# luisdavid64/MRI-Implicit-Neural-Representations

Measured on AMD Instinct MI355X. Metric: coord-samples/sec (fwd+bwd) fitting 640x368x15-coil k-space; PSNR@1k steps, higher is better.
Workload: dtype f32; 1 GPU; SIREN 5x256 gauss-512 k-space fit, synthetic 640x368x15-coil, L2, Adam; batch_per_gpu=25000, global_batch=25000, parallelism=single, launch=eager

## Files before the change

mri-implicit-neural-representations_amd/csrc/inr_mlp_rs_impl.h:

```cpp
#pragma once
#include "inr_mlp_impl.h"

namespace inr {

constexpr int RS_PITCH = 132;
constexpr int RS_IMG_FLOATS = 256 * RS_PITCH;
constexpr int RS_CP = 32;
constexpr int RS_CHUNK_FLOATS = 2 * RS_CP * RS_PITCH;
constexpr int RS_CHUNK_STEPS = 2 * RS_CP / 4;
constexpr int RS_PF = 8;
constexpr int RS_LR = 8;
constexpr int RS_OOB = 0x7ffffff0;
constexpr int RS_HSZ = 256 * 128;

typedef float f32x2 __attribute__((ext_vector_type(2)));
typedef unsigned u32x2 __attribute__((ext_vector_type(2)));
typedef __attribute__((address_space(3))) float lfloat;
typedef __attribute__((address_space(3))) f32x4 lf32x4;

__device__ __forceinline__ f32x4 mfma16(float a, float b, f32x4 c) {
  return __builtin_amdgcn_mfma_f32_16x16x4f32(a, b, c, 0, 0, 0);
}

template <int NCB>
__device__ __forceinline__ int rs_tl(int c, int jj) {
  return ((NCB & 1) && c == NCB - 1) ? 16 * (NCB - 1) + jj : 32 * (c >> 1) + 2 * jj + (c & 1);
}
template <int NCB>
__device__ __forceinline__ bool rs_active(int c, int n) {
  return ((NCB & 1) && c == NCB - 1) ? n == NCB : (c | 1) < n;
}

template <int NCB>
struct RsAddr {
  static constexpr int NP = (NCB + 1) / 2;
  __amdgpu_buffer_rsrc_t rs;
  int cB[NP];
  int cC[NP];
};

__device__ __forceinline__ void rs_store2(__amdgpu_buffer_rsrc_t rs, int voff, int soff, float x, float y) {
  u32x2 v = {__builtin_bit_cast(unsigned, x), __builtin_bit_cast(unsigned, y)};
  __builtin_amdgcn_raw_buffer_store_b64(v, rs, voff, soff, 0);
}
__device__ __forceinline__ void rs_store1(__amdgpu_buffer_rsrc_t rs, int voff, int soff, float x) {
  __builtin_amdgcn_raw_buffer_store_b32(__builtin_bit_cast(unsigned, x), rs, voff, soff, 0);
}
__device__ __forceinline__ f32x2 rs_load2(__amdgpu_buffer_rsrc_t rs, int voff, int soff) {
  return __builtin_bit_cast(f32x2, __builtin_amdgcn_raw_buffer_load_b64(rs, voff, soff, 0));
}
__device__ __forceinline__ float rs_load1(__amdgpu_buffer_rsrc_t rs, int voff, int soff) {
  return __builtin_bit_cast(float, __builtin_amdgcn_raw_buffer_load_b32(rs, voff, soff, 0));
}

__device__ __forceinline__ float rs_dk_put(bool in_agpr, float v) {
  if (!in_agpr) return v;
  float a;
  asm("v_accvgpr_write_b32 %0, %1" : "=a"(a) : "v"(v));
  return a;
}
__device__ __forceinline__ float rs_dk_get(bool in_agpr, float a) {
  if (!in_agpr) return a;
  float v;
  asm("v_accvgpr_read_b32 %0, %1" : "=v"(v) : "a"(a));
  return v;
}
template <int NCB>
constexpr bool rs_dk_agpr(int rb, int reg) { return true; }

__device__ __forceinline__ float rs_bval(const f32x4& b0, const f32x4& b1, int c) { return c < 4 ? b0[c] : b1[c - 4]; }

template <int NCB>
__device__ __forceinline__ void rs_store_brows(const RsAddr<NCB>& ad, int soff, const f32x4& b0, const f32x4& b1) {
  constexpr int NP = RsAddr<NCB>::NP;
#pragma unroll
  for (int p = 0; p < NP; ++p) {
    if ((NCB & 1) && p == NP - 1)
      rs_store1(ad.rs, ad.cB[p], soff, rs_bval(b0, b1, 2 * p));
    else
      rs_store2(ad.rs, ad.cB[p], soff, rs_bval(b0, b1, 2 * p), rs_bval(b0, b1, 2 * p + 1));
  }
}

template <int NCB>
__device__ __forceinline__ void rs_store_crow(const RsAddr<NCB>& ad, int soff, const f32x4 (&v)[2]) {
  constexpr int NP = RsAddr<NCB>::NP;
#pragma unroll
  for (int p = 0; p < NP; ++p) {
    if ((NCB & 1) && p == NP - 1)
      rs_store1(ad.rs, ad.cC[p], soff, v[(2 * p) >> 2][(2 * p) & 3]);
    else
      rs_store2(ad.rs, ad.cC[p], soff, v[(2 * p) >> 2][(2 * p) & 3], v[(2 * p + 1) >> 2][(2 * p + 1) & 3]);
  }
}

#define RS_KIND_FEAT 1
#define RS_KIND_FWD 2
#define RS_KIND_BWD 3

template <int NCB, int NSTEPS, int KIND, int INIT>
__device__ __forceinline__ void rs_gemm(f32x4 (&acc)[4][NCB], f32x4 (&Ar)[RS_PF], const __amdgpu_buffer_rsrc_t ars,
                                        const int avoff, const int asoff, const int asoff_next, const lfloat* Bl,
                                        const RsAddr<NCB>& ad, const int w, const int soffB, const int soffB2,
                                        f32x2 (&dk)[4][4][(NCB + 1) / 2], const int soffD, const f32x4 (&cinit)[4]) {
  constexpr int NP = (NCB + 1) / 2;
  constexpr int NQ = (NCB + 3) / 4;
  static_assert(NSTEPS % RS_PF == 0, "the fragment ring must be in phase at the start of every GEMM");
  f32x2 lr[RS_LR];
  f32x4 b0, b1 = {0.f, 0.f, 0.f, 0.f};
  b0 = *(const lf32x4*)(Bl);
  if (NQ > 1) b1 = *(const lf32x4*)(Bl + 4);
  const lfloat* Blw = Bl + w * 4 * RS_PITCH;
  f32x4 st0, st1 = {0.f, 0.f, 0.f, 0.f};
  st0 = *(const lf32x4*)(Blw);
  if (NQ > 1) st1 = *(const lf32x4*)(Blw + 4);
#pragma unroll
  for (int s = 0; s < NSTEPS; ++s) {
    const f32x4 afr = Ar[s % RS_PF];
    {
      const int so = s + RS_PF < NSTEPS ? asoff + (s + RS_PF) * 4096 : asoff_next + (s + RS_PF - NSTEPS) * 4096;
      Ar[s % RS_PF] = __builtin_bit_cast(f32x4, __builtin_amdgcn_raw_buffer_load_b128(ars, avoff, so, 0));
    }
    f32x4 n0 = b0, n1 = b1;
    if (s + 1 < NSTEPS) {
      n0 = *(const lf32x4*)(Bl + (s + 1) * 4 * RS_PITCH);
      if (NQ > 1) n1 = *(const lf32x4*)(Bl + (s + 1) * 4 * RS_PITCH + 4);
    }
    if ((s & 3) == 0) {
      const int rowb = KIND == RS_KIND_FEAT ? (s < NSTEPS / 2 ? soffB + 4 * s * 512 : soffB2 + 4 * (s - NSTEPS / 2) * 512)
                                            : soffB + 4 * s * 512;
      rs_store_brows<NCB>(ad, rowb + w * 2048, st0, st1);
    }
    if ((s & 3) == 3 && s + 1 < NSTEPS) {
      st0 = *(const lf32x4*)(Blw + (s + 1) * 4 * RS_PITCH);
      if (NQ > 1) st1 = *(const lf32x4*)(Blw + (s + 1) * 4 * RS_PITCH + 4);
    }
    if (KIND == RS_KIND_FWD || KIND == RS_KIND_BWD) {
      constexpr int TOT = 16 * NP;
      const int j0 = s * TOT / NSTEPS, j1 = (s + 1) * TOT / NSTEPS;
#pragma unroll
      for (int j = j0; j < j1; ++j) {
        const int rr = j / NP, p = j % NP, rb = rr >> 2, reg = rr & 3;
        const int so = soffD + (16 * rb + reg) * 512;
        const bool single = (NCB & 1) && p == NP - 1;
        if (KIND == RS_KIND_FWD) {
          if (single)
            rs_store1(ad.rs, ad.cC[p], so, rs_dk_get(rs_dk_agpr<NCB>(rb, reg), dk[rb][reg][p][0]));
          else
            rs_store2(ad.rs, ad.cC[p], so, rs_dk_get(rs_dk_agpr<NCB>(rb, reg), dk[rb][reg][p][0]),
                      rs_dk_get(rs_dk_agpr<NCB>(rb, reg), dk[rb][reg][p][1]));
        } else {
          if (j >= RS_LR) {
            const int jo = j - RS_LR, ro = jo / NP, po = jo % NP;
            dk[ro >> 2][ro & 3][po][0] = rs_dk_put(rs_dk_agpr<NCB>(ro >> 2, ro & 3), lr[jo % RS_LR][0]);
            if (!((NCB & 1) && po == NP - 1))
              dk[ro >> 2][ro & 3][po][1] = rs_dk_put(rs_dk_agpr<NCB>(ro >> 2, ro & 3), lr[jo % RS_LR][1]);
          }
          if (single) {
            lr[j % RS_LR][0] = rs_load1(ad.rs, ad.cC[p], so);
            lr[j % RS_LR][1] = 0.f;
          } else {
            lr[j % RS_LR] = rs_load2(ad.rs, ad.cC[p], so);
          }
        }
      }
    }
#pragma unroll
    for (int c = 0; c < NCB; ++c) {
      const float bv = rs_bval(b0, b1, c);
#pragma unroll
      for (int rb = 0; rb < 4; ++rb)
        acc[rb][c] = mfma16(afr[rb], bv,
                            (INIT == 1 && s == 0) ? f32x4{0.f, 0.f, 0.f, 0.f} : ((INIT == 2 && s == 0) ? cinit[rb] : acc[rb][c]));
    }
#pragma unroll
    for (int i = 0; i < 12; ++i) {
      __builtin_amdgcn_sched_group_barrier(0x008, 1, 0);
      __builtin_amdgcn_sched_group_barrier(0x1b6, 1, 0);
    }
    __builtin_amdgcn_sched_barrier(0);
    b0 = n0;
    b1 = n1;
  }
  if (KIND == RS_KIND_BWD) {
    constexpr int TOT = 16 * NP;
#pragma unroll
    for (int jo = TOT - RS_LR; jo < TOT; ++jo) {
      const int ro = jo / NP, po = jo % NP;
      dk[ro >> 2][ro & 3][po][0] = rs_dk_put(rs_dk_agpr<NCB>(ro >> 2, ro & 3), lr[jo % RS_LR][0]);
      if (!((NCB & 1) && po == NP - 1))
        dk[ro >> 2][ro & 3][po][1] = rs_dk_put(rs_dk_agpr<NCB>(ro >> 2, ro & 3), lr[jo % RS_LR][1]);
    }
  }
}

template <int NCB>
__device__ __forceinline__ void rs_gen(lfloat* buf, const lfloat* encB_lds, int ch, const float (&xs)[NCB][3], int tid) {
  const int jj = tid & 15, p0 = tid >> 4;
#pragma unroll
  for (int i = 0; i < 2; ++i) {
    const int p = p0 + 16 * i, s = ch * RS_CP + p;
    const float e0 = encB_lds[3 * s + 0], e1 = encB_lds[3 * s + 1], e2 = encB_lds[3 * s + 2];
    f32x4 sn[2] = {{0.f, 0.f, 0.f, 0.f}, {0.f, 0.f, 0.f, 0.f}}, cs[2] = {{0.f, 0.f, 0.f, 0.f}, {0.f, 0.f, 0.f, 0.f}};
#pragma unroll
    for (int c = 0; c < NCB; ++c) {
      const float ph = fmaf(xs[c][2], e2, fmaf(xs[c][1], e1, xs[c][0] * e0));
      float a, b;
      sincos_cw(ph, a, b);
      sn[c >> 2][c & 3] = a;
      cs[c >> 2][c & 3] = b;
    }
    lfloat* q = buf + p * RS_PITCH + jj * 8;
    *(lf32x4*)(q) = sn[0];
    *(lf32x4*)(q + RS_CP * RS_PITCH) = cs[0];
    if (NCB > 4) {
      *(lf32x4*)(q + 4) = sn[1];
      *(lf32x4*)(q + RS_CP * RS_PITCH + 4) = cs[1];
    }
  }
}

template <int HACT>
__device__ __forceinline__ float rs_act_park(float z, float w0, float& h) {
  if (HACT == ACT_SIN) {
    constexpr float c_hi = 0.15915494309189535f;
    constexpr float c_lo = (float)(0.15915494309189533576888 - (double)c_hi);
    const float t = w0 * z;
    const float k = rintf(t * c_hi);
    const float rev = fmaf(t, c_lo, fmaf(t, c_hi, -k));
    h = __builtin_amdgcn_sinf(rev);
    return rev;
  }
  float d;
  act_fwd<HACT>(z, w0, h, d);
  return z;
}
template <int HACT>
__device__ __forceinline__ void rs_act_unpark(float p, float w0, float& h, float& d) {
  if (HACT == ACT_SIN) {
    h = __builtin_amdgcn_sinf(p);
    d = w0 * __builtin_amdgcn_cosf(p);
  } else {
    act_fwd<HACT>(p, w0, h, d);
  }
}

template <int NCB, int HACT>
struct RsLast {
  lfloat *wl_lds, *dzl, *red, *part, *Cl;
  float* slab;
  bool lvalid, sampled, first;
  long long lrow;
  int w, kq, jj, tid, lane;

  template <int MO>
  __device__ __forceinline__ float run(const NetDesc& nd, const LossDesc& ld, const MlpArgs& a, const f32x4 (&acc)[4][NCB],
                                       const float (&gt_pre)[4], const float (&lb_pre)[4], float w0) {
    constexpr int NQ = (NCB + 3) / 4;
    constexpr int NW = 4;
    (void)NW;
    const LayerDesc& LL = nd.L[nd.D - 1];
    float loss = 0.f;
    f32x4 yp[MO][2];
#pragma unroll
    for (int o = 0; o < MO; ++o) yp[o][0] = yp[o][1] = f32x4{0.f, 0.f, 0.f, 0.f};
#pragma unroll
    for (int rb = 0; rb < 4; ++rb) {
      f32x4 wv[MO];
#pragma unroll
      for (int o = 0; o < MO; ++o) wv[o] = *(const lf32x4*)(wl_lds + o * 256 + 64 * w + 16 * rb + 4 * kq);
#pragma unroll
      for (int reg = 0; reg < 4; ++reg) {
        f32x4 hq[2] = {{0.f, 0.f, 0.f, 0.f}, {0.f, 0.f, 0.f, 0.f}}, pq[2] = {{0.f, 0.f, 0.f, 0.f}, {0.f, 0.f, 0.f, 0.f}};
#pragma unroll
        for (int c = 0; c < NCB; ++c) {
          float h;
          pq[c >> 2][c & 3] = rs_act_park<HACT>(acc[rb][c][reg], w0, h);
          hq[c >> 2][c & 3] = h;
        }
#pragma unroll
        for (int q = 0; q < NQ; ++q) {
          *(lf32x4*)(Cl + (16 * rb + reg) * RS_PITCH + 4 * q) = pq[q];
#pragma unroll
          for (int o = 0; o < MO; ++o) yp[o][q] += wv[o][reg] * hq[q];
        }
        __builtin_amdgcn_sched_barrier(0);
      }
    }
    INR_STAMP(50);
#pragma unroll
    for (int o = 0; o < MO; ++o)
#pragma unroll
      for (int q = 0; q < 2; ++q)
#pragma unroll
        for (int e = 0; e < 4; ++e) {
          float v = yp[o][q][e];
          v += __shfl_xor(v, 16);
          v += __shfl_xor(v, 32);
          yp[o][q][e] = v;
        }
    if (kq == 0) {
#pragma unroll
      for (int o = 0; o < MO; ++o) {
        lfloat* pp = part + (w * MO + o) * 128 + jj * 8;
        *(lf32x4*)pp = yp[o][0];
        *(lf32x4*)(pp + 4) = yp[o][1];
      }
    }
    INR_STAMP(51);
    __syncthreads();
    INR_STAMP(52);
    if (tid < 128) {
      float zl[4], y[4], dy[4], g[4] = {0.f, 0.f, 0.f, 0.f}, dz[4] = {0.f, 0.f, 0.f, 0.f};
#pragma unroll
      for (int o = 0; o < 4; ++o) {
        float s = 0.f;
        if (o < MO)
          s = ((part[o * 128 + tid] + part[(MO + o) * 128 + tid]) + part[(2 * MO + o) * 128 + tid]) +
              part[(3 * MO + o) * 128 + tid];
        zl[o] = o < nd.out_f ? s + lb_pre[o] : 0.f;
      }
      const int nrows = nd.out_f;
#pragma unroll
      for (int o = 0; o < 4; ++o) {
        y[o] = dy[o] = 0.f;
        if (o < nd.out_f) act_fwd_rt(nd.last_act, zl[o], nd.w0, y[o], dy[o]);
      }
      if (lvalid) {
#pragma unroll
        for (int o = 0; o < 4; ++o)
          if (o < nd.out_f && a.out != nullptr) a.out[lrow * nd.out_f + o] = y[o];
        if (sampled) loss = loss_row(ld, nd.out_f, y, gt_pre, g);
#pragma unroll
        for (int o = 0; o < 4; ++o)
          if (o < nrows) dz[o] = g[o] * dy[o];
      }
#pragma unroll
      for (int o = 0; o < MO; ++o) dzl[o * 128 + tid] = dz[o];
    }
    INR_STAMP(53);
    __syncthreads();
    INR_STAMP(54);
    f32x4 dzv[MO][2];
#pragma unroll
    for (int o = 0; o < MO; ++o)
#pragma unroll
      for (int q = 0; q < 2; ++q)
        dzv[o][q] = q < NQ ? *(const lf32x4*)(dzl + o * 128 + jj * 8 + 4 * q) : f32x4{0.f, 0.f, 0.f, 0.f};
    const __amdgpu_buffer_rsrc_t rsb = uniform_rsrc(slab + LL.gb_off, LL.M * 4);
    float db_mine, dw_mine[4];
    {
      float sb[MO];
#pragma unroll
      for (int o = 0; o < MO; ++o) {
        sb[o] = 0.f;
#pragma unroll
        for (int c = 0; c < NCB; ++c) sb[o] += dzv[o][c >> 2][c & 3];
      }
      group_sum_n<16, MO>(sb);
      float mine = sb[0];
#pragma unroll
      for (int o = 1; o < MO; ++o) mine = jj == o ? sb[o] : mine;
      db_mine = mine;
    }
    const __amdgpu_buffer_rsrc_t rsw = uniform_rsrc(slab + LL.gw_off, LL.M * LL.K * 4);
    {
      f32x4 nx[2] = {{0.f, 0.f, 0.f, 0.f}, {0.f, 0.f, 0.f, 0.f}};
#pragma unroll
      for (int q = 0; q < NQ; ++q) nx[q] = *(const lf32x4*)(Cl + 4 * q);
      f32x4 wv[MO];
      float pw[MO * 4];
#pragma unroll
      for (int rr = 0; rr < 16; ++rr) {
        const int rb = rr >> 2, reg = rr & 3;
        lfloat* row = Cl + (16 * rb + reg) * RS_PITCH;
        if (reg == 0) {
#pragma unroll
          for (int o = 0; o < MO; ++o) wv[o] = *(const lf32x4*)(wl_lds + o * 256 + 64 * w + 16 * rb + 4 * kq);
        }
        f32x4 hq[2] = {nx[0], nx[1]}, dq[2] = {{0.f, 0.f, 0.f, 0.f}, {0.f, 0.f, 0.f, 0.f}};
        f32x4 dd[2] = {{0.f, 0.f, 0.f, 0.f}, {0.f, 0.f, 0.f, 0.f}};
        if (rr + 1 < 16) {
#pragma unroll
          for (int q = 0; q < NQ; ++q)
            nx[q] = *(const lf32x4*)(Cl + (16 * ((rr + 1) >> 2) + ((rr + 1) & 3)) * RS_PITCH + 4 * q);
        }
#pragma unroll
        for (int c = 0; c < NCB; ++c) {
          float h, d;
          rs_act_unpark<HACT>(hq[c >> 2][c & 3], w0, h, d);
          hq[c >> 2][c & 3] = h;
          dd[c >> 2][c & 3] = d;
        }
#pragma unroll
        for (int o = 0; o < MO; ++o) {
          float sp = 0.f;
#pragma unroll
          for (int c = 0; c < NCB; ++c) sp = fmaf(dzv[o][c >> 2][c & 3], hq[c >> 2][c & 3], sp);
          pw[o * 4 + reg] = sp;
        }
#pragma unroll
        for (int c = 0; c < NCB; ++c) {
          float sd = 0.f;
#pragma unroll
          for (int o = 0; o < MO; ++o) sd = fmaf(wv[o][reg], dzv[o][c >> 2][c & 3], sd);
          dq[c >> 2][c & 3] = sd * dd[c >> 2][c & 3];
        }
#pragma unroll
        for (int q = 0; q < NQ; ++q) *(lf32x4*)(row + 4 * q) = dq[q];
        if (reg == 3) {
          group_sum_n<16, MO * 4>(pw);
          float mine = pw[0];
#pragma unroll
          for (int i = 1; i < MO * 4; ++i) mine = jj == i ? pw[i] : mine;
          dw_mine[rb] = mine;
        }
        __builtin_amdgcn_sched_barrier(0);
      }
    }
    {
      const int so_ = jj >> 2;
      int off[5];
#pragma unroll
      for (int rb = 0; rb < 4; ++rb) {
        const int rowi = 64 * w + 16 * rb + 4 * kq + (jj & 3);
        off[rb] = (jj < MO * 4 && so_ < LL.M && rowi < LL.K) ? (so_ * LL.K + rowi) * 4 : RS_OOB;
      }
      off[4] = (w == 0 && kq == 0 && jj < MO && jj < LL.M) ? jj * 4 : RS_OOB;
      if (!first) {
        float old[5];
#pragma unroll
        for (int rb = 0; rb < 4; ++rb) old[rb] = rs_load1(rsw, off[rb], 0);
        old[4] = rs_load1(rsb, off[4], 0);
#pragma unroll
        for (int rb = 0; rb < 4; ++rb) dw_mine[rb] += old[rb];
        db_mine += old[4];
      }
#pragma unroll
      for (int rb = 0; rb < 4; ++rb) rs_store1(rsw, off[rb], 0, dw_mine[rb]);
      rs_store1(rsb, off[4], 0, db_mine);
    }
    INR_STAMP(55);
    return loss;
  }
};

template <int NCB, int HACT>
__global__ __launch_bounds__(256) void inr_mlp_rs_kernel(const NetDesc nd, const LossDesc ld, const MlpArgs a) {
  extern __shared__ __attribute__((aligned(16))) float lds[];
  constexpr int NW = 4;
  (void)NW;
  constexpr int NP = (NCB + 1) / 2;
  constexpr int NQ = (NCB + 3) / 4;
  const int tid = threadIdx.x, lane = tid & 63;
  const int w = __builtin_amdgcn_readfirstlane(tid >> 6);
  INR_RT_STAMP(a.dbg, a.dbg_cap, NW, w, lane, 44);
  const int kq = lane >> 4, jj = lane & 15;
  const int D = nd.D, E = nd.E;
  lfloat* img = (lfloat*)lds;
  lfloat* encB_lds = img + RS_IMG_FLOATS;
  lfloat* wl_lds = encB_lds + ((3 * E + 3) & ~3);
  lfloat* dzl = wl_lds + 1024;
  lfloat* red = dzl + 512;
  lfloat* part = red + 32;
  const LayerDesc& LL = nd.L[D - 1];
  for (int i = tid; i < 3 * E; i += 256) encB_lds[i] = a.encB[i];
  for (int i = tid; i < 1024; i += 256) {
    const int o = i >> 8, k = i & 255;
    wl_lds[i] = (o < LL.M && k < LL.K) ? a.params[LL.w_off + o * LL.K + k] : 0.f;
  }
  float* slab = a.slabs + (size_t)blockIdx.x * nd.slab_floats;
  float loss_acc = 0.f;
  if (((int)blockIdx.x < a.rs_x ? a.rs_hi : a.rs_lo) == 0 && a.accumulate == 0) {
    for (int i = tid; i < LL.M * LL.K; i += 256) slab[LL.gw_off + i] = 0.f;
    if (tid < LL.M) slab[LL.gb_off + tid] = 0.f;
  }
  const long long spt = nd.save_floats_per_tile;
  const __amdgpu_buffer_rsrc_t ars = uniform_rsrc(a.packed, 0x7ffffff0);
  const int avoff = lane * 16 + w * 1024;
  const lfloat* Bl = img + kq * RS_PITCH + jj * 8;
  lfloat* Cl = img + (64 * w + 4 * kq) * RS_PITCH + jj * 8;
  const int enc_off = (2 * (D - 1) * RS_HSZ + 4 * 128) * 4;
  const int nch = E / RS_CP;
  f32x4 Ar[RS_PF];
  {
    const int so = nd.L[0].rf_off * 4;
#pragma unroll
    for (int i = 0; i < RS_PF; ++i)
      Ar[i] = __builtin_bit_cast(f32x4, __builtin_amdgcn_raw_buffer_load_b128(ars, avoff, so + i * 4096, 0));
  }

  for (int r = 0; r < a.rs_rounds; ++r) {
    const int t = r * gridDim.x + blockIdx.x;
    const int n = t < a.rs_x ? a.rs_hi : a.rs_lo;
    const int blk0 = t < a.rs_x ? t * a.rs_hi : a.rs_x * a.rs_hi + (t - a.rs_x) * a.rs_lo;
    if (n == 0) continue;
    const bool first = r == 0 && a.accumulate == 0;
    const long long g0 = (long long)blk0 * 16;
    const int slot0 = blk0 >> 3;
    RsAddr<NCB> ad;
    {
      const int nslots = a.n_tiles - slot0 < 2 ? a.n_tiles - slot0 : 2;
      ad.rs = uniform_rsrc(a.save + (size_t)slot0 * spt, (int)(nslots * spt * 4));
#pragma unroll
      for (int p = 0; p < NP; ++p) {
        const int gl = (blk0 & 7) * 16 + rs_tl<NCB>(2 * p, jj);
        const int off = (int)(((gl >> 7) * spt + (gl & 127)) * 4);
        const bool act = rs_active<NCB>(2 * p, n);
        ad.cB[p] = act ? off + kq * 512 : RS_OOB;
        ad.cC[p] = act ? off + kq * 2048 : RS_OOB;
      }
    }
    float xs[NCB][3];
#pragma unroll
    for (int c = 0; c < NCB; ++c) {
      const long long g = g0 + rs_tl<NCB>(c, jj);
      const bool ok = rs_active<NCB>(c, n) && g < a.B;
      const float two_pi = 6.283185307179586f;
#pragma unroll
      for (int i = 0; i < 3; ++i) xs[c][i] = ok ? two_pi * a.x[3 * g + i] : 0.f;
    }
    float gt_pre[4] = {0.f, 0.f, 0.f, 0.f}, lb_pre[4] = {0.f, 0.f, 0.f, 0.f};
    bool sampled_pre = false, lvalid = false;
    long long lrow = 0;
    if (tid < 128) {
      const int cq = tid & 7, jq = tid >> 3;
      if (cq < NCB) {
        lrow = g0 + rs_tl<NCB>(cq, jq);
        lvalid = rs_active<NCB>(cq, n) && lrow < a.B;
      }
#pragma unroll
      for (int o = 0; o < 4; ++o)
        if (o < nd.out_f) lb_pre[o] = a.packed[LL.pbias_off + o];
      if (lvalid) {
        sampled_pre = a.mask == nullptr || a.mask[lrow] != 0;
#pragma unroll
        for (int o = 0; o < 4; ++o)
          if (o < nd.out_f) gt_pre[o] = a.gt[lrow * nd.out_f + o];
      }
    }
    INR_STAMP(0);
    __syncthreads();
    f32x4 acc[4][NCB];
    f32x2 dk[4][4][NP];
    f32x4 bnext[4];
#pragma unroll
    for (int rb = 0; rb < 4; ++rb) {
      bnext[rb] = *reinterpret_cast<const f32x4*>(a.packed + nd.L[0].pbias_off + 64 * w + 4 * kq + 16 * rb);
#pragma unroll
      for (int c = 0; c < NCB; ++c) acc[rb][c] = bnext[rb];
    }
    rs_gen<NCB>(img, encB_lds, 0, xs, tid);
    __syncthreads();
    for (int ch = 0; ch < nch; ++ch) {
      if (ch == 1) INR_STAMP(56);
      if (ch + 1 < nch) rs_gen<NCB>(img + ((ch + 1) & 1) * RS_CHUNK_FLOATS, encB_lds, ch + 1, xs, tid);
      if (ch == 1) INR_STAMP(57);
      const int ao = (nd.L[0].rf_off + ch * RS_CHUNK_STEPS * 1024) * 4;
      const int an = ch + 1 < nch ? ao + RS_CHUNK_STEPS * 4096 : (D > 2 ? nd.L[1].rf_off : nd.L[0].rf_off) * 4;
      const int sb = enc_off + ch * RS_CP * 512;
      rs_gemm<NCB, RS_CHUNK_STEPS, RS_KIND_FEAT, 0>(acc, Ar, ars, avoff, ao, an, Bl + (ch & 1) * RS_CHUNK_FLOATS, ad, w, sb,
                                                    sb + E * 512, dk, 0, bnext);
      if (ch == 1) INR_STAMP(58);
      __syncthreads();
      if (ch == 1) INR_STAMP(59);
    }
    INR_STAMP(1);
    for (int l = 1; l <= D - 2; ++l) {
      {
#pragma unroll
        for (int rb = 0; rb < 4; ++rb)
          bnext[rb] = *reinterpret_cast<const f32x4*>(a.packed + nd.L[l].pbias_off + 64 * w + 4 * kq + 16 * rb);
        const float w0 = nd.L[l - 1].omega;
#pragma unroll
        for (int rb = 0; rb < 4; ++rb) {
#pragma unroll
          for (int reg = 0; reg < 4; ++reg) {
            f32x4 hq[2] = {{0.f, 0.f, 0.f, 0.f}, {0.f, 0.f, 0.f, 0.f}};
#pragma unroll
            for (int c = 0; c < NCB; ++c) {
              float h, d;
              act_fwd<HACT>(acc[rb][c][reg], w0, h, d);
              hq[c >> 2][c & 3] = h;
              dk[rb][reg][c >> 1][c & 1] = rs_dk_put(rs_dk_agpr<NCB>(rb, reg), d);
            }
#pragma unroll
            for (int q = 0; q < NQ; ++q) *(lf32x4*)(Cl + (16 * rb + reg) * RS_PITCH + 4 * q) = hq[q];
            __builtin_amdgcn_sched_barrier(0);
          }
        }
      }
      if (l == 1) INR_STAMP(60);
      __syncthreads();
      INR_STAMP(20 + l - 1);
      const LayerDesc& Ll = nd.L[l];
      const int an = l < D - 2 ? nd.L[l + 1].rf_off * 4 : nd.L[D - 2].rb_off * 4;
      rs_gemm<NCB, 64, RS_KIND_FWD, 2>(acc, Ar, ars, avoff, Ll.rf_off * 4, an, Bl, ad, w, (2 * (l - 1)) * RS_HSZ * 4, 0, dk,
                                       ((2 * (l - 1) + 1) * RS_HSZ + 64 * w * 128) * 4, bnext);
      INR_STAMP(1 + l);
      __syncthreads();
      if (l == 1) INR_STAMP(61);
    }
    INR_STAMP(10);
    {
      RsLast<NCB, HACT> ls{wl_lds, dzl, red, part, Cl, slab, lvalid, sampled_pre, first, lrow, w, kq, jj, tid, lane};
      if (LL.M > 2)
        loss_acc += ls.template run<4>(nd, ld, a, acc, gt_pre, lb_pre, nd.L[D - 2].omega);
      else
        loss_acc += ls.template run<2>(nd, ld, a, acc, gt_pre, lb_pre, nd.L[D - 2].omega);
    }
    __syncthreads();
    INR_STAMP(20 + D - 2);
    INR_STAMP(11);
    for (int l = D - 2; l >= 1; --l) {
      const LayerDesc& Ll = nd.L[l];
      const int an = (l > 1 ? nd.L[l - 1].rb_off : nd.L[0].rf_off) * 4;
      rs_gemm<NCB, 64, RS_KIND_BWD, 1>(acc, Ar, ars, avoff, Ll.rb_off * 4, an, Bl, ad, w, (2 * l + 1) * RS_HSZ * 4, 0, dk,
                                       ((2 * (l - 1) + 1) * RS_HSZ + 64 * w * 128) * 4, bnext);
      INR_STAMP(12 + l);
      if (l > 1) {
        __syncthreads();
#pragma unroll
        for (int rb = 0; rb < 4; ++rb)
#pragma unroll
          for (int reg = 0; reg < 4; ++reg) {
            f32x4 dq[2] = {{0.f, 0.f, 0.f, 0.f}, {0.f, 0.f, 0.f, 0.f}};
#pragma unroll
            for (int c = 0; c < NCB; ++c) dq[c >> 2][c & 3] = acc[rb][c][reg] * rs_dk_get(rs_dk_agpr<NCB>(rb, reg), dk[rb][reg][c >> 1][c & 1]);
#pragma unroll
            for (int q = 0; q < NQ; ++q) *(lf32x4*)(Cl + (16 * rb + reg) * RS_PITCH + 4 * q) = dq[q];
          }
        __syncthreads();
        INR_STAMP(30 + l);
      }
    }
    {
      const int so0 = (1 * RS_HSZ + 64 * w * 128) * 4;
#pragma unroll
      for (int rb = 0; rb < 4; ++rb)
#pragma unroll
        for (int reg = 0; reg < 4; ++reg) {
          f32x4 dq[2] = {{0.f, 0.f, 0.f, 0.f}, {0.f, 0.f, 0.f, 0.f}};
          if (D > 2) {
#pragma unroll
            for (int c = 0; c < NCB; ++c) dq[c >> 2][c & 3] = acc[rb][c][reg] * rs_dk_get(rs_dk_agpr<NCB>(rb, reg), dk[rb][reg][c >> 1][c & 1]);
          } else {
#pragma unroll
            for (int q = 0; q < NQ; ++q) dq[q] = *(const lf32x4*)(Cl + (16 * rb + reg) * RS_PITCH + 4 * q);
          }
          rs_store_crow<NCB>(ad, so0 + (16 * rb + reg) * 512, dq);
        }
    }
    INR_STAMP(40);
  }

  {
    float v = loss_acc;
#pragma unroll
    for (int off = 32; off >= 1; off >>= 1) v += __shfl_xor(v, off);
    __syncthreads();
    if (lane == 0) red[w] = v;
    __syncthreads();
    if (tid == 0) {
      const float tsum = ((red[0] + red[1]) + red[2]) + red[3];
      slab[nd.slab_loss_off] = a.accumulate ? slab[nd.slab_loss_off] + tsum : tsum;
    }
  }
  INR_RT_STAMP(a.dbg, a.dbg_cap, NW, w, lane, 45);
}

inline size_t rs_lds_bytes(const NetDesc& nd) {
  return ((size_t)RS_IMG_FLOATS + ((3 * (size_t)nd.E + 3) & ~(size_t)3) + 1024 + 512 + 32 + 2048) * sizeof(float);
}

template <int NCB, int HACT>
inline hipError_t launch_mlp_rs(const NetDesc& nd, const LossDesc& ld, const MlpArgs& a, int grid, hipStream_t st) {
  const size_t lds_bytes = rs_lds_bytes(nd);
  if (lds_bytes > 160 * 1024) return hipErrorInvalidValue;
  hipError_t e = allow_full_lds<inr_mlp_rs_kernel<NCB, HACT>>();
  if (e != hipSuccess) return e;
  hipLaunchKernelGGL((inr_mlp_rs_kernel<NCB, HACT>), dim3(grid), dim3(256), lds_bytes, st, nd, ld, a);
  return hipGetLastError();
}

}
```

Measured before the change: 61.45 million coord-samples/s.

## Interleave Fourier feature generation into layer-0 MFMA loop

Moves the sin/cos Gaussian-feature generation for the next chunk out of a separate rs_gen pass and into the layer-0 GEMM step loop. Each step computes a share of the features and writes them into the other LDS buffer, with scheduling barriers that pair MFMAs with VALU/LDS ops so transcendental work hides under matrix ops. On the last chunk it harmlessly regenerates the current chunk into the spare buffer. It adds register pressure and more complex scheduling inside the hot GEMM, which may reduce occupancy or disturb the tuned pipeline.

```diff
diff --git a/mri-implicit-neural-representations_amd/csrc/inr_mlp_rs_impl.h b/mri-implicit-neural-representations_amd/csrc/inr_mlp_rs_impl.h
--- a/mri-implicit-neural-representations_amd/csrc/inr_mlp_rs_impl.h
+++ b/mri-implicit-neural-representations_amd/csrc/inr_mlp_rs_impl.h
@@ -98,14 +98,39 @@
 #define RS_KIND_FWD 2
 #define RS_KIND_BWD 3
 
-template <int NCB, int NSTEPS, int KIND, int INIT>
+template <int NCB>
+struct RsGen {
+  int other;
+  const lfloat* enc;
+  float xs[NCB][3];
+};
+
+__device__ __forceinline__ void rs_feat(const float (&x)[3], float e0, float e1, float e2, float& sn, float& cs) {
+  const float ph = fmaf(x[2], e2, fmaf(x[1], e1, x[0] * e0));
+  sincos_cw(ph, sn, cs);
+}
+
+template <int NCB, int NSTEPS, int KIND, int INIT, bool GEN = false>
 __device__ __forceinline__ void rs_gemm(f32x4 (&acc)[4][NCB], f32x4 (&Ar)[RS_PF], const __amdgpu_buffer_rsrc_t ars,
                                         const int avoff, const int asoff, const int asoff_next, const lfloat* Bl,
                                         const RsAddr<NCB>& ad, const int w, const int soffB, const int soffB2,
-                                        f32x2 (&dk)[4][4][(NCB + 1) / 2], const int soffD, const f32x4 (&cinit)[4]) {
+                                        f32x2 (&dk)[4][4][(NCB + 1) / 2], const int soffD, const f32x4 (&cinit)[4],
+                                        const RsGen<NCB>* gen = nullptr) {
   constexpr int NP = (NCB + 1) / 2;
   constexpr int NQ = (NCB + 3) / 4;
   static_assert(NSTEPS % RS_PF == 0, "the fragment ring must be in phase at the start of every GEMM");
+  static_assert(!GEN || KIND == RS_KIND_FEAT, "only layer 0 generates features");
+  float ge[2][3] = {{0.f, 0.f, 0.f}, {0.f, 0.f, 0.f}};
+  f32x4 gsn = {0.f, 0.f, 0.f, 0.f}, gcs = {0.f, 0.f, 0.f, 0.f};
+  if (GEN) {
+    int gl;
+    asm volatile("v_mbcnt_lo_u32_b32 %0, -1, 0\n\tv_mbcnt_hi_u32_b32 %0, -1, %0" : "=v"(gl));
+    const lfloat* ep = gen->enc + 3 * (4 * w + (gl >> 4));
+#pragma unroll
+    for (int i = 0; i < 2; ++i)
+#pragma unroll
+      for (int k = 0; k < 3; ++k) ge[i][k] = ep[3 * 16 * i + k];
+  }
   f32x2 lr[RS_LR];
   f32x4 b0, b1 = {0.f, 0.f, 0.f, 0.f};
   b0 = *(const lf32x4*)(Bl);
@@ -165,6 +190,24 @@
         }
       }
     }
+    if (GEN) {
+      constexpr int TOT = 2 * NCB, GS = NSTEPS - 1;
+      const int u0 = s < GS ? s * TOT / GS : TOT, u1 = s + 1 < GS ? (s + 1) * TOT / GS : TOT;
+#pragma unroll
+      for (int u = u0; u < u1; ++u) {
+        const int i = u / NCB, c = u % NCB;
+        if ((c & 3) == 0) gsn = gcs = f32x4{0.f, 0.f, 0.f, 0.f};
+        float sn, cs;
+        rs_feat(gen->xs[c], ge[i][0], ge[i][1], ge[i][2], sn, cs);
+        gsn[c & 3] = sn;
+        gcs[c & 3] = cs;
+        if ((c & 3) == 3 || c == NCB - 1) {
+          lfloat* q = (lfloat*)Blw + gen->other + 16 * i * RS_PITCH + (c & ~3);
+          *(lf32x4*)(q) = gsn;
+          *(lf32x4*)(q + RS_CP * RS_PITCH) = gcs;
+        }
+      }
+    }
 #pragma unroll
     for (int c = 0; c < NCB; ++c) {
       const float bv = rs_bval(b0, b1, c);
@@ -173,10 +216,18 @@
         acc[rb][c] = mfma16(afr[rb], bv,
                             (INIT == 1 && s == 0) ? f32x4{0.f, 0.f, 0.f, 0.f} : ((INIT == 2 && s == 0) ? cinit[rb] : acc[rb][c]));
     }
-#pragma unroll
-    for (int i = 0; i < 12; ++i) {
-      __builtin_amdgcn_sched_group_barrier(0x008, 1, 0);
-      __builtin_amdgcn_sched_group_barrier(0x1b6, 1, 0);
+    if (GEN) {
+#pragma unroll
+      for (int i = 0; i < (4 * NCB > 12 ? 4 * NCB : 12); ++i) {
+        __builtin_amdgcn_sched_group_barrier(0x008, 1, 0);
+        __builtin_amdgcn_sched_group_barrier(0x5b6, 1, 0);
+      }
+    } else {
+#pragma unroll
+      for (int i = 0; i < 12; ++i) {
+        __builtin_amdgcn_sched_group_barrier(0x008, 1, 0);
+        __builtin_amdgcn_sched_group_barrier(0x1b6, 1, 0);
+      }
     }
     __builtin_amdgcn_sched_barrier(0);
     b0 = n0;
@@ -204,9 +255,8 @@
     f32x4 sn[2] = {{0.f, 0.f, 0.f, 0.f}, {0.f, 0.f, 0.f, 0.f}}, cs[2] = {{0.f, 0.f, 0.f, 0.f}, {0.f, 0.f, 0.f, 0.f}};
 #pragma unroll
     for (int c = 0; c < NCB; ++c) {
-      const float ph = fmaf(xs[c][2], e2, fmaf(xs[c][1], e1, xs[c][0] * e0));
       float a, b;
-      sincos_cw(ph, a, b);
+      rs_feat(xs[c], e0, e1, e2, a, b);
       sn[c >> 2][c & 3] = a;
       cs[c >> 2][c & 3] = b;
     }
@@ -511,7 +561,8 @@
         ad.cC[p] = act ? off + kq * 2048 : RS_OOB;
       }
     }
-    float xs[NCB][3];
+    RsGen<NCB> gen;
+    float (&xs)[NCB][3] = gen.xs;
 #pragma unroll
     for (int c = 0; c < NCB; ++c) {
       const long long g = g0 + rs_tl<NCB>(c, jj);
@@ -554,13 +605,15 @@
     __syncthreads();
     for (int ch = 0; ch < nch; ++ch) {
       if (ch == 1) INR_STAMP(56);
-      if (ch + 1 < nch) rs_gen<NCB>(img + ((ch + 1) & 1) * RS_CHUNK_FLOATS, encB_lds, ch + 1, xs, tid);
       if (ch == 1) INR_STAMP(57);
+      const int chg = ch + 1 < nch ? ch + 1 : ch;
+      gen.other = (ch & 1) ? -RS_CHUNK_FLOATS : RS_CHUNK_FLOATS;
+      gen.enc = encB_lds + 3 * chg * RS_CP;
       const int ao = (nd.L[0].rf_off + ch * RS_CHUNK_STEPS * 1024) * 4;
       const int an = ch + 1 < nch ? ao + RS_CHUNK_STEPS * 4096 : (D > 2 ? nd.L[1].rf_off : nd.L[0].rf_off) * 4;
       const int sb = enc_off + ch * RS_CP * 512;
-      rs_gemm<NCB, RS_CHUNK_STEPS, RS_KIND_FEAT, 0>(acc, Ar, ars, avoff, ao, an, Bl + (ch & 1) * RS_CHUNK_FLOATS, ad, w, sb,
-                                                    sb + E * 512, dk, 0, bnext);
+      rs_gemm<NCB, RS_CHUNK_STEPS, RS_KIND_FEAT, 0, true>(acc, Ar, ars, avoff, ao, an, Bl + (ch & 1) * RS_CHUNK_FLOATS, ad, w,
+                                                          sb, sb + E * 512, dk, 0, bnext, &gen);
       if (ch == 1) INR_STAMP(58);
       __syncthreads();
       if (ch == 1) INR_STAMP(59);
```

New measurement: 61.09 million coord-samples/s. No clear change (-0.6%).
